# eazuooz/RayTracinginOneWeekendinCUDA

Measured on AMD Instinct MI355X. Metric: Msamples/s (pixels x spp / s), whole job, higher is better.
Workload: dtype f64; 1 GPU; C2 Book-1 final random-spheres, HittableList world (no BVH), 1200x800x500spp x50 bounces; frames_in_flight=1, width=1200, height=800, spp=500, max_depth=50, seed=1984, variant=strict, rng=XORWOW (cuRAND device-API semantics), one sequence per pixel

## Files before the change

### include/rtow.h

```cpp
#ifndef RTOW_H
#define RTOW_H

#include <stddef.h>
#include <stdint.h>

#ifdef __cplusplus
extern "C" {
#endif

#define RTOW_API __attribute__((visibility("default")))

typedef uint32_t rt_handle;
typedef struct rt_scene rt_scene;
typedef struct rt_rng rt_rng;
typedef struct rt_film rt_film;

enum rt_status {
    RT_OK = 0,
    RT_ERR_INVALID = 1,
    RT_ERR_UNSUPPORTED = 2,
    RT_ERR_HIP = 3,
    RT_ERR_NO_DEVICE = 4,
    RT_ERR_STATE = 5
};
// ... 73 lines not shown
    uint32_t n_nodes;
    uint32_t n_spheres, n_moving_spheres, n_quads;
    uint32_t n_objects;
    uint32_t n_xforms, n_media, n_materials, n_textures, n_perlin, n_images;
    uint32_t table_bytes;
    uint32_t image_bytes;
    uint32_t reserved[3];
} rt_scene_info;
RTOW_API int rt_scene_get_info(rt_scene *s, rt_scene_info *out);

RTOW_API int rt_scene_dump_leaves(rt_scene *s, int max_leaves, int *kind_out, double *box_out);
RTOW_API int rt_scene_dump_nodes(rt_scene *s, int max_nodes, double *box_out, uint32_t *abe_out);
RTOW_API int rt_scene_dump_fast_nodes(rt_scene *s, int max_nodes, double *box_out, uint32_t *ab_out, uint16_t *link_out);
RTOW_API int rt_scene_dump_camera(rt_scene *s, double out27[27]);
RTOW_API int rt_scene_dump_scan_segments(rt_scene *s, int max_segments, uint32_t *rows_axis_out, float *shared_out);

typedef struct rt_render_params {
    int32_t width, height;
    int32_t samples_per_pixel;
    int32_t max_depth;
    uint64_t seed;
    int32_t stripe_rows;
    int32_t rank, world_size;
    int32_t variant;
    int32_t device;
    int32_t flags;
    void *stream;
    int32_t coop_threshold;
    int32_t overdue_rays_per_sample;
    int32_t shade_batch;
    int32_t max_blocks_per_cu;
    int32_t pixels_per_wave;
    int32_t reserved0;
} rt_render_params;

#define RT_FLAG_KEEP_RNG_STATE 1u
#define RT_FLAG_OVERDUE_PRIORITY 4u
#define RT_FLAG_ACCUMULATE 8u
#define RT_FLAG_FORCE_GENERAL 2u
#define RT_FLAG_ALWAYS_WALK 32u
#define RT_FLAG_NO_PIXEL_CLASSES 64u
#define RT_FLAG_REFERENCE_TREE 128u
#define RT_FLAG_EXACT_SCAN 256u
#define RT_FLAG_FILTER_FP64 2048u
#define RT_FLAG_ACCELERATE_LISTS 512u
#define RT_FLAG_COOP_SINGLE 1024u
#define RT_FLAG_ROW_MAJOR_TILES 16u

typedef struct rt_render_stats {
    uint64_t samples;
    uint64_t rays;
    double seconds_seed;
    double seconds_render;
    uint32_t pixels;
    uint32_t rows;
    uint32_t kernel_vgprs;
    uint32_t lds_bytes;
    uint32_t kernel_kind;
    uint32_t pixels_per_wave;
// ... 158 lines not shown
```

### raytracinginoneweekendincuda_amd/__init__.py

```python
from .api import (
    RtowError,
    Rng,
    Scene,
    Film,
    RenderParams,
    RenderStats,
    LaunchPlan,
    builtin_scene,
    stripe_rows,
    deinterleave,
    write_ppm,
    write_ppm_binary,
    write_pfm,
    rtwimage_bytes,
    load_image,
    load_obj,
    jpeg_decode,
    library_path,
    lib,
    AdaptiveParams,
    adaptive_converged,
    adaptive_rule_on_device,
    FLAG_KEEP_RNG_STATE,
    FLAG_FORCE_GENERAL,
    FLAG_OVERDUE_PRIORITY,
    FLAG_ACCUMULATE,
    FLAG_ROW_MAJOR_TILES,
    FLAG_ALWAYS_WALK, FLAG_NO_PIXEL_CLASSES, FLAG_REFERENCE_TREE, FLAG_EXACT_SCAN, FLAG_ACCELERATE_LISTS, FLAG_COOP_SINGLE, FLAG_FILTER_FP64,
    SCENE_PLAIN_QUADS, SCENE_REFERENCE_TREE_ONLY,
)

__all__ = [
    "RtowError", "Rng", "Scene", "Film", "RenderParams", "RenderStats", "builtin_scene",
    "stripe_rows", "deinterleave", "write_ppm", "write_ppm_binary", "write_pfm", "rtwimage_bytes", "load_image", "load_obj", "library_path", "lib",
    "FLAG_KEEP_RNG_STATE", "FLAG_FORCE_GENERAL", "FLAG_OVERDUE_PRIORITY", "FLAG_ACCUMULATE", "FLAG_ROW_MAJOR_TILES", "FLAG_ALWAYS_WALK",
    "AdaptiveParams", "adaptive_converged", "adaptive_rule_on_device",
]
```

### raytracinginoneweekendincuda_amd/_lib.py

```python
import ctypes as C
import os

_HERE = os.path.dirname(os.path.abspath(__file__))
LIB_PATH = os.environ.get("RTOW_LIB_PATH") or os.path.join(_HERE, "librtow_hip.so")


class RenderParams(C.Structure):
    _fields_ = [
        ("width", C.c_int32), ("height", C.c_int32), ("samples_per_pixel", C.c_int32), ("max_depth", C.c_int32),
        ("seed", C.c_uint64), ("stripe_rows", C.c_int32), ("rank", C.c_int32), ("world_size", C.c_int32),
        ("variant", C.c_int32), ("device", C.c_int32), ("flags", C.c_int32), ("stream", C.c_void_p),
        ("coop_threshold", C.c_int32), ("overdue_rays_per_sample", C.c_int32),
        ("shade_batch", C.c_int32), ("max_blocks_per_cu", C.c_int32), ("pixels_per_wave", C.c_int32), ("reserved0", C.c_int32),
    ]


class RenderStats(C.Structure):
    _fields_ = [
        ("samples", C.c_uint64), ("rays", C.c_uint64), ("seconds_seed", C.c_double), ("seconds_render", C.c_double),
        ("pixels", C.c_uint32), ("rows", C.c_uint32), ("kernel_vgprs", C.c_uint32), ("lds_bytes", C.c_uint32),
        ("kernel_kind", C.c_uint32), ("pixels_per_wave", C.c_uint32),
    ]


# ... 126 lines not shown
    "rt_hittable_list": (H, [P, C.POINTER(H), I]),
    "rt_constant_medium": (H, [P, H, D, D, D, D]),
    "rt_constant_medium_tex": (H, [P, H, D, H]),
    "rt_bvh_node": (H, [P, C.POINTER(H), I]),
    "rt_hittable_bounding_box": (I, [P, H, D3]),
    "rt_scene_set_world": (I, [P, H]),
    "rt_scene_set_camera": (I, [P, D3, D3, D3, D, D, D, D, D, D, D3]),
    "rt_scene_build_builtin": (I, [P, I, I, I, I, C.c_uint64, P, I, I]),
    "rt_scene_commit": (I, [P]),
    "rt_scene_get_info": (I, [P, C.POINTER(SceneInfo)]),
    "rt_scene_dump_leaves": (I, [P, I, C.POINTER(C.c_int), D3]),
    "rt_scene_dump_nodes": (I, [P, I, D3, C.POINTER(C.c_uint32)]),
    "rt_scene_dump_fast_nodes": (I, [P, I, D3, C.POINTER(C.c_uint32), C.POINTER(C.c_uint16)]),
    "rt_scene_dump_camera": (I, [P, D3]),
    "rt_scene_dump_scan_segments": (I, [P, I, C.POINTER(C.c_uint32), C.POINTER(C.c_float)]),
    "rt_stripe_rows": (I, [I, I, I, I, C.POINTER(C.c_int), I]),
    "rt_film_create": (P, [I, I, I, I, I, I]),
    "rt_film_destroy": (None, [P]),
    "rt_film_device_pixels": (P, [P]),
    "rt_film_pixel_bytes": (C.c_size_t, [P]),
    "rt_film_bind_pixels": (I, [P, P]),
    "rt_plan_launch": (I, [P, C.POINTER(RenderParams), I, I, C.POINTER(LaunchPlan)]),
    "rt_film_download_probe_costs": (I, [P, C.POINTER(C.c_uint32), I, I]),
    "rt_scene_upload": (I, [P, I]),
    "rt_render_launch": (I, [P, P, C.POINTER(RenderParams)]),
    "rt_render_finish": (I, [P, P, C.POINTER(RenderStats)]),
    "rt_film_download": (I, [P, D3, I, I]),
    "rt_film_set_adaptive": (I, [P, C.POINTER(AdaptiveParams)]),
    "rt_film_download_sample_counts": (I, [P, C.POINTER(C.c_uint32), I, I]),
    "rt_adaptive_converged": (I, [C.POINTER(AdaptiveParams), C.c_uint32, D, D, D, D]),
# ... 44 lines not shown
```

### raytracinginoneweekendincuda_amd/api.py

```python
import ctypes as C
import numbers

import numpy as np

from . import _lib
from ._lib import (AdaptiveParams, DenoiseParams, FeatureParams, LaunchPlan, QueryHits, QueryParams, QueryRays, QueryStats,
                   RadianceOut, RadianceParams, RadianceRays, RadianceStats, RenderParams, RenderStats, SceneInfo)


class RtowError(RuntimeError):
    pass


FLAG_KEEP_RNG_STATE = 1
FLAG_FORCE_GENERAL = 2
FLAG_OVERDUE_PRIORITY = 4
FLAG_ACCUMULATE = 8
FLAG_ROW_MAJOR_TILES = 16
FLAG_ALWAYS_WALK = 32
FLAG_ACCELERATE_LISTS = 512
FLAG_EXACT_SCAN = 256
FLAG_REFERENCE_TREE = 128
FLAG_FILTER_FP64 = 2048
FLAG_COOP_SINGLE = 1024
FLAG_NO_PIXEL_CLASSES = 64


SCENE_PLAIN_QUADS = 1
SCENE_REFERENCE_TREE_ONLY = 2


DENOISE_DEFAULTS = {"iterations": 5, "sigma_color": 0.6, "sigma_albedo": 0.1, "sigma_normal": 0.3, "sigma_depth": 0.1}


def lib():
    return _lib.load()


def library_path():
# ... 199 lines not shown
        return boxes[:n], ab[:n], links[:n]

    def dump_camera(self):
        out = np.zeros(27, dtype=np.float64)
        _check(lib().rt_scene_dump_camera(self._p, out.ctypes.data_as(_lib.D3)))
        return out

    def scan_segments(self):
        n = lib().rt_scene_dump_scan_segments(self._p, 0, None, None)
        if n < 0:
            raise RtowError(_err())
        rows = np.zeros((max(n, 1), 3), dtype=np.uint32)
        shared = np.zeros(max(n, 1), dtype=np.float32)
        lib().rt_scene_dump_scan_segments(self._p, n, rows.ctypes.data_as(C.POINTER(C.c_uint32)), shared.ctypes.data_as(C.POINTER(C.c_float)))
        return [(int(r[0]), int(r[1]), None if r[2] == 3 else int(r[2]), shared[k]) for k, r in enumerate(rows[:n])]

    def plan_launch(self, params, num_cus=256, adaptive=False):
        out = LaunchPlan()
        _check(lib().rt_plan_launch(self._p, C.byref(params), num_cus, 1 if adaptive else 0, C.byref(out)))
        plan = {n: getattr(out, n) for n, _ in LaunchPlan._fields_ if not n.startswith("lds_table_")}
        plan["lds_tables"] = {name: (None if off == _lib.LDS_GLOBAL else off, size)
                              for name, off, size in zip(_lib.LDS_TABLES, out.lds_table_offset, out.lds_table_bytes)}
        return plan

    def upload(self, device=0):
        _check(lib().rt_scene_upload(self._p, device))

    def _ray_batch(self, kind, origins, directions, inputs, outputs, want, calls, structs, stats, device):
        on_gpu = type(origins).__module__.split(".")[0] == "torch"
        if on_gpu:
# ... 322 lines not shown
```

### raytracinginoneweekendincuda_amd/csrc/device_scene.cpp

```cpp
#include <hip/hip_runtime.h>

#include <cstdio>
#include <cmath>
#include <cstring>
#include <initializer_list>
#include <map>
#include <mutex>
#include <string>
#include <vector>

#include "../../include/rtow.h"
#include "device_arena.h"
#include "film_rows.h"
#include "launch_plan.h"
#include "render_iface.h"
#include "scene_host.h"

namespace rtow {

static int hip_fail(hipError_t e, const char *what)
{
    return fail(RT_ERR_HIP, std::string("HIP error = ") + std::to_string((unsigned)e) + " (" + hipGetErrorString(e) +
                                ") at '" + what + "'");
}
#define HIP_TRY(expr)                                     \
    do {                                                  \
        hipError_t e_ = (expr);                           \
        if (e_ != hipSuccess) return hip_fail(e_, #expr); \
    } while (0)
// ... 44 lines not shown
    DeviceArena planes;
    size_t plane_pixels() const { return geometry.n_pixels ? geometry.n_pixels : 1; }
    double *pixels = nullptr;
    double *own_pixels = nullptr;
    double *accum = nullptr;
    int accum_spp = 0;
    double *carry = nullptr;
    uint32_t *state = nullptr;
    unsigned long long *ray_counter = nullptr;
    int num_cus = 256;
    hipStream_t own_stream = nullptr;
    hipStream_t last_stream = nullptr;
    uint32_t *tile_cost = nullptr, *tile_order = nullptr;
    uint32_t *pix_cost = nullptr, *heavy_list = nullptr, *heavy_count = nullptr, *super_list = nullptr;
    uint8_t *pix_class = nullptr;
    unsigned long long *host_counters = nullptr;
    hipEvent_t ev[4] = {nullptr, nullptr, nullptr, nullptr};
    bool seeded = false;
    bool in_flight = false;
    SceneImpl *scene_in_flight = nullptr;
    uint64_t last_samples = 0;
    int last_variant = 0;
    rt_launch_plan last_plan{};
    KernelInfo last_kernel{};
    bool adaptive = false, frame_adaptive = false, last_adaptive = false;
    AdaptiveRule rule{}, frame_rule{};
    uint32_t *ad_n = nullptr;
    double *ad_q = nullptr;
    uint8_t *ad_mark = nullptr;
    bool rendered = false;
// ... 273 lines not shown
    f->geometry = film_geometry(width, height, stripe_rows, rank, world_size);
    const size_t np = f->plane_pixels();
    hipError_t e = f->planes.alloc(np * 3, f->own_pixels);
    if (e == hipSuccess) e = hipMemset(f->own_pixels, 0, np * 3 * sizeof(double));
    f->pixels = f->own_pixels;
    if (e == hipSuccess) e = f->planes.alloc(np * 6, f->state);
    if (e == hipSuccess) e = f->planes.alloc(kCounterWords, f->ray_counter);
    if (e == hipSuccess) {
        hipDeviceProp_t prop;
        e = hipGetDeviceProperties(&prop, device);
        if (e == hipSuccess) f->num_cus = prop.multiProcessorCount;
    }
    if (e == hipSuccess) e = hipStreamCreateWithFlags(&f->own_stream, hipStreamNonBlocking);
    if (e == hipSuccess) e = f->planes.alloc(f->geometry.n_tiles, f->tile_cost);
    if (e == hipSuccess) e = f->planes.alloc(f->geometry.n_tiles, f->tile_order);
    if (e == hipSuccess) e = hipHostMalloc((void **)&f->host_counters, kCounterWords * sizeof(unsigned long long), hipHostMallocDefault);
    for (int k = 0; k < 4 && e == hipSuccess; k++) e = hipEventCreate(&f->ev[k]);
    if (e != hipSuccess) {
        hip_fail(e, "rt_film_create allocation");
        rt_film_destroy(reinterpret_cast<rt_film *>(f));
        return nullptr;
    }
    return reinterpret_cast<rt_film *>(f);
}

void rt_film_destroy(rt_film *film)
{
    if (!film) return;
    FilmImpl *f = F(film);
    hipSetDevice(f->device);
// ... 219 lines not shown
    HIP_TRY(hipEventRecord(f.ev[0], stream));
    if (!keep)
        if (int rc = seed_film(f, p, stream)) return rc;
    HIP_TRY(hipEventRecord(f.ev[1], stream));
    RenderArgs ra{};
    if (int rc = book_frame(f, p, keep, continues, ra, stream)) return rc;
    const rt_launch_plan plan = plan_launch(ds, f.geometry, f.num_cus, *p, f.adaptive, hits_stay_in_boxes(s.flat, s.camera, p->variant));
    fill_render_args(f, p, plan, ra);
    KernelInfo info{};
    HIP_TRY(build.info(plan.kernel, ds, ra, &info));
    if (info.kind != plan.kernel_kind || info.lds_bytes != plan.lds_bytes)
        return fail(RT_ERR_STATE, "rt_render_launch: the kernel is not the one the launch plan describes");
    f.last_plan = plan;
    f.last_kernel = info;
    if (int rc = allocate_class_planes(f, plan)) return rc;
    if (plan.probe_spp > 0)
        if (int rc = enqueue_rehearsal(f, ds, plan, build, ra, stream)) return rc;
    HIP_TRY(build.render(plan.kernel, ds, ra, stream));
    HIP_TRY(hipEventRecord(f.ev[2], stream));
    HIP_TRY(hipMemcpyAsync(f.host_counters, f.ray_counter, kCounterWords * sizeof(unsigned long long), hipMemcpyDeviceToHost, stream));
    HIP_TRY(hipEventRecord(f.ev[3], stream));
    return RT_OK;
}

int rt_render_launch(rt_scene *scene, rt_film *film, const rt_render_params *p)
{
    if (!scene || !film || !p) return fail(RT_ERR_INVALID, "rt_render_launch: null argument");
    SceneImpl &s = *S(scene);
    FilmImpl &f = *F(film);
    if (p->width != f.geometry.width || p->height != f.geometry.height || p->stripe_rows != f.stripe_rows || p->rank != f.rank ||
// ... 38 lines not shown
                            "box pass", "medium pass / between walks", "object pass", "primitive pass", "  hit record", "  scatter",
                            "  next camera ray", "  pixel done"};
    if (is_sphere_list_kernel(f.last_kernel.kind)) {
        name[0] = "scan, pixel-parallel";
        name[1] = "scan, cooperative";
        name[12] = name[13] = "";
        const double passes = (double)c[96 + 0], groups = (double)c[96 + 12], taken = (double)c[64 + 12];
        if (groups > 0) {
            std::fprintf(stderr, "survivors: %.0f passes, %.2f groups of 4 per pass, groups taken f = %.4f\n", passes, groups / passes, taken / groups);
            std::fprintf(stderr, "survivors: spheres with a passing lane per taken group %.3f, lane appends per pass %.1f, lanes behind per pass %.2f\n",
                         (double)c[32 + 12] / taken, (double)c[96 + 13] / passes, (double)c[64 + 13] / passes);
            std::fprintf(stderr, "survivors: drains per pass %.2f, drain iterations (wave max of count) per pass %.2f, drain cycles %.1f %% of the "
                         "pixel-parallel scan's (%.0f of %.0f per pass)\n", (double)c[96 + 15] / passes, (double)c[64 + 15] / passes,
                         100.0 * c[32 + 13] / c[32 + 0], (double)c[32 + 13] / passes, (double)c[32 + 0] / passes);
        }
        name[16] = name[17] = name[18] = "";
        const double gp = (double)c[96 + 16];
        if (gp > 0) {
            std::fprintf(stderr, "grouped: %.0f passes through the filter, %.2f rays per pass, exact-test blocks executed per pass %.2f\n", gp,
                         (double)c[64 + 16] / gp, (double)c[32 + 16] / gp);
            std::fprintf(stderr, "grouped: survivors (lanes tested) per pass %.2f, largest per-lane count per pass %.2f, drains per pass %.2f\n",
                         (double)c[32 + 17] / gp, (double)c[64 + 17] / gp, (double)c[96 + 17] / gp);
            std::fprintf(stderr, "grouped: cycles per pass: filter %.0f, exact tests %.0f (%.1f %% and %.1f %% of the cooperative scans' %.0f)\n",
                         (double)c[64 + 18] / gp, (double)c[32 + 18] / gp, 100.0 * c[64 + 18] / c[32 + 1], 100.0 * c[32 + 18] / c[32 + 1],
                         (double)c[32 + 1] / (double)c[96 + 1]);
        }
    }
    const double total = (double)c[7];
    for (int k = 0; k < 24; k++)
        if (name[k][0] && c[96 + k])
// ... 448 lines not shown
```

### raytracinginoneweekendincuda_amd/csrc/render.hip

```cpp
#include <hip/hip_runtime.h>

#include <cfloat>
#include <cstddef>
#include <cstdint>
#include <type_traits>

#include "flat_scene.h"
#include "launch_plan.h"
#include "render_iface.h"
#include "rng.h"

#ifndef RT_STRICT
#define RT_STRICT 1
#endif
#ifndef RT_GROUP
#define RT_GROUP 0
#endif
#ifndef RT_ADAPT
#define RT_ADAPT 0
#endif
#ifndef RT_FEATURES
#define RT_FEATURES 0
#endif
#ifndef RT_QUERY
// ... 1431 lines not shown
    const double bu = f.od - s;
    return bu > f.root_m && __builtin_fma(bu, bu, k - q) > 0.0;
}

DEV SphereScanRow load_scan_row(const SphereScanRow *table, uint32_t k)
{
    const RT_CONST double *p = const_doubles(table + k);
    return SphereScanRow{p[0], p[1], p[2], p[3]};
}
DEV void scan_rows_arrived(const SphereScanRow &g0, const SphereScanRow &g1, const SphereScanRow &g2, const SphereScanRow &g3)
{
    asm volatile("" ::"s"(g0.cx), "s"(g0.cy), "s"(g0.cz), "s"(g0.k), "s"(g1.cx), "s"(g1.cy), "s"(g1.cz), "s"(g1.k));
    asm volatile("" ::"s"(g2.cx), "s"(g2.cy), "s"(g2.cz), "s"(g2.k), "s"(g3.cx), "s"(g3.cy), "s"(g3.cz), "s"(g3.k));
}

constexpr int kFilterTrip = 8;
static_assert(kFilterTrip < kQueueCap, "a trip of appends must fit between the drain threshold and the end of the queue");
DEV void append_survivor(uint16_t *queue, uint32_t lane, uint32_t &count, uint32_t k, bool keep)
{
    queue[count * 64u + lane] = (uint16_t)k;
    count += keep ? 1u : 0u;
}

DEV void filter_four(const SphereScanRow &g0, const SphereScanRow &g1, const SphereScanRow &g2, const SphereScanRow &g3, uint32_t k0,
                     const ScanRay &f, uint16_t *queue, uint32_t lane, uint32_t &count)
{
    const SphereScanRow *g[4] = {&g0, &g1, &g2, &g3};
    double s[4], q[4];
#pragma unroll
    for (int u = 0; u < 4; u++) {
// ... 1357 lines not shown
    int i = 0, j = 0;
    size_t local = 0;
    Xorwow rng{0, 0, 0, 0, 0, 0};
    Vec col = mk(0.0, 0.0, 0.0);
    Vec throughput = mk(1.0, 1.0, 1.0), accumulated = mk(0.0, 0.0, 0.0);
    Ray ray{};
    int sample = 0, depth = 0;
    uint32_t wave_rays = 0;
    [[maybe_unused]] uint32_t ad_before = 0;
    [[maybe_unused]] double ad_q = 0.0;
    [[maybe_unused]] unsigned long long wave_samples = 0;

    uint32_t pix_rays = 0;
    uint32_t my_tile = 0;
    int boost_left = 0;
    Walk walk{};
    walk.state = kNone;
    HitInfo walk_best;
    walk_best.t = 0.0;
    walk_best.ref = kNone;
    walk_best.obj = kNone;
    [[maybe_unused]] SegState seg{0u, kSegEnd, 0u};

    const uint32_t probe_cap = (!T::ADAPTIVE && a.probe && a.probe_ray_cap > 0) ? (uint32_t)a.probe_ray_cap : 0xFFFFFFFFu;
    auto book_cost = [&](uint32_t rays) {
        if constexpr (T::PARK) {
            local = (size_t)park_get_int<T::BLOCK>(sc.lds_park, 2);
            const uint32_t row = (uint32_t)local / (uint32_t)a.width, column = (uint32_t)local % (uint32_t)a.width;
            my_tile = (row >> 3) * tiles_x + (column >> 3);
        }
// ... 4 lines not shown
#if RT_PHASES
    PhaseSums ph{};
    const unsigned long long ph_start = __builtin_readcyclecounter();
    bool ph_serving = heavy_mode;
#endif
    for (;;) {
        unsigned long long overdue = 0;
        bool boost = false;
        if constexpr (T::WORLD == 2) {
            overdue = __ballot(active && pix_rays >= a.ray_budget);
            if (a.overdue_priority) {
                if (overdue) __builtin_amdgcn_s_setprio(3);
                else __builtin_amdgcn_s_setprio(0);
                overdue = 0;
            }
            boost = overdue != 0 && boost_left > 0;
            if (boost) boost_left--;
            else boost_left = a.boost_rounds;
        }

        const bool from_list = heavy_mode && !heavy_dry;
        if (solo_hold && !__any(active)) solo_hold = false;
        if (!exhausted && !boost && (!heavy_mode || from_list) && !solo_hold) {
            unsigned long long need = __ballot(!active);
            const bool from_super = from_list && solo_phase;
            const int ppw = from_super ? super_ppw : (from_list ? heavy_ppw : a.pixels_per_wave);
            if (ppw < 64) need &= (1ull << ppw) - 1ull;
            if (need) {
                PH_BEGIN();
                [[maybe_unused]] const bool ph_was_idle = !active;
                const uint32_t cnt = (uint32_t)__popcll(need);
                const uint32_t queue_len = from_super ? super_total : (from_list ? heavy_total : total_slots);
                uint32_t base = 0;
// ... 90 lines not shown
#endif
                continue;
            }
            if (exhausted) break;
            continue;
        }

        unsigned long long todo = live;
        HitInfo h;
        h.t = 0.0;
        h.ref = kNone;
        h.obj = kNone;
        bool hit = false;
        if constexpr (T::WORLD == 2) {
            if (boost) todo = overdue;
            if (!boost && a.pixels_per_wave >= 64 && __popcll(live) >= a.coop_threshold) {
                PH_BEGIN();
#if RT_PHASES
                ScanSums ss{};
#endif
                if (active) hit = a.exact_scan    ? scan_uniform(sc, queue, lane, ray, 0.001, DBL_MAX, h)
                                 : a.filter_fp64 ? (sv.in_lds ? scan_filtered<true>(sc, sv.planes_off, sv.n_padded, queue, lane, ray, 0.001, DBL_MAX, h SS_PASS)
                                                              : scan_filtered<false>(sc, 0u, 0u, queue, lane, ray, 0.001, DBL_MAX, h SS_PASS))
                                 : sv.in_lds     ? scan_filtered32<true>(sc, sv.planes_off, sv.n_padded, queue, lane, ray, 0.001, DBL_MAX, h SS_PASS)
                                                 : scan_filtered32<false>(sc, 0u, 0u, queue, lane, ray, 0.001, DBL_MAX, h SS_PASS);
                PH_END(0, active);
#if RT_PHASES
                {
                    const int src = __ffsll((long long)__ballot(active)) - 1;
                    if (src >= 0) {
                    const auto rl = [src](uint32_t v) { return (unsigned long long)(uint32_t)__builtin_amdgcn_readlane((int)v, src); };
                    ph.n[12] += rl(ss.groups);  ph.l[12] += rl(ss.taken);        ph.t[12] += rl(ss.spheres);
                    ph.n[13] += rl(ss.appends); ph.l[13] += rl(ss.behind);       ph.t[13] += rl(ss.drain_cycles);
                    ph.n[15] += rl(ss.drains);  ph.l[15] += rl(ss.drain_iters);
                    }
                }
#endif
            } else {
                PH_BEGIN();
#if RT_PHASES
                GroupedSums gs{};
#endif
// ... 386 lines not shown
    klass[k] = heavy ? 1 : 0;
    if (longest) super_list[atomicAdd(count + 1, 1u)] = k;
    else if (heavy) list[atomicAdd(count, 1u)] = k;
}

hipError_t launch_classify_pixels(const uint32_t *pix_cost, uint32_t n_pixels, uint32_t threshold, uint8_t *pix_class, uint32_t *list,
                                  uint32_t *count, hipStream_t stream, uint32_t *super_list, uint32_t super_threshold, uint32_t width,
                                  uint32_t near_percent, uint32_t near_neighbours)
{
    if (n_pixels == 0) return hipSuccess;
    hipLaunchKernelGGL(classify_pixels_kernel, dim3((n_pixels + 255u) / 256u), dim3(256), 0, stream, pix_cost, n_pixels, threshold,
                       pix_class, list, count, super_list, super_threshold, width, near_percent, near_neighbours);
    return hipGetLastError();
}

hipError_t launch_tile_order(const uint32_t *tile_cost, uint32_t *tile_order, uint32_t n_tiles, uint32_t flat_x8, hipStream_t stream)
{
    if (n_tiles == 0) return hipSuccess;
    hipLaunchKernelGGL(tile_order_kernel, dim3(1), dim3(1024), 0, stream, tile_cost, tile_order, n_tiles, flat_x8);
    return hipGetLastError();
}
#endif

#if RT_STRICT
#define RT_SUFFIX strict
#else
#define RT_SUFFIX fast
#endif
#define RT_CAT2(a, b) a##b
#define RT_CAT(a, b) RT_CAT2(a, b)
// ... 581 lines not shown
```

### raytracinginoneweekendincuda_amd/csrc/render_iface.h

```cpp
#pragma once
#include <hip/hip_runtime.h>

#include <cstdint>

#include "adaptive_rule.h"
#include "flat_scene.h"
#include "rng.h"

namespace rtow {

struct SeedArgs {
    uint32_t *state;
    const uint32_t *jump_table;
    Xorwow base;
    uint32_t *tile_cost;
    const uint32_t *tile_order;
    int32_t probe;
    uint32_t n_pixels;
    int32_t width, stripe_rows, rank, world_size;
};

struct RenderArgs {
    double *pixels;
    double *accum;
// ... 32 lines not shown
    int32_t exact_scan;
    int32_t filter_fp64;
    int32_t reference_tree;
    int32_t always_walk;
    int32_t force_general;
    int32_t coop_threshold;
    int32_t coop_single;
    int32_t num_cus;
    int32_t lds_spheres;
    int32_t overdue_priority;
    int32_t boost_rounds;
    int32_t max_blocks_per_cu;
    int32_t pixels_per_wave;
    int32_t shade_batch;
    uint32_t ray_budget;
    int32_t adaptive;
    AdaptiveRule rule;
    uint32_t *ad_n;
    double *ad_q;
    uint8_t *ad_mark;
};

struct KernelInfo {
    int vgprs, lds_bytes, kind;
};

hipError_t launch_seed_strict(const SeedArgs &a, hipStream_t stream);
hipError_t launch_seed_fast(const SeedArgs &a, hipStream_t stream);
hipError_t launch_render_strict(int kernel, const DeviceScene &sc, const RenderArgs &a, hipStream_t stream);
hipError_t launch_render_fast(int kernel, const DeviceScene &sc, const RenderArgs &a, hipStream_t stream);
// ... 59 lines not shown

struct AtrousArgs {
    const double *in;
    double *out;
    const double *albedo, *normal;
    const double *depth;
    int32_t width, height, step;
    double inv_color, inv_albedo, inv_normal, inv_depth;
};
hipError_t launch_atrous(const AtrousArgs &a, hipStream_t stream);

hipError_t launch_classify_pixels(const uint32_t *pix_cost, uint32_t n_pixels, uint32_t threshold, uint8_t *pix_class, uint32_t *list,
                                  uint32_t *count, hipStream_t stream, uint32_t *super_list = nullptr, uint32_t super_threshold = 0,
                                  uint32_t width = 0, uint32_t near_percent = 0, uint32_t near_neighbours = 0);

hipError_t launch_tile_order(const uint32_t *tile_cost, uint32_t *tile_order, uint32_t n_tiles, uint32_t flat_x8, hipStream_t stream);

}
```

### raytracinginoneweekendincuda_amd/csrc/scene_builder.cpp

```cpp
#include <algorithm>
#include <cfloat>
#include <charconv>
#include <cmath>
#include <limits>
#include <cstdio>
#include <cstdlib>
#include <cstring>
#include <mutex>
#include <unordered_map>

#include "../../include/rtow.h"
#include "scene_host.h"

namespace rtow {

static thread_local std::string g_error;
void set_error(const std::string &msg) { g_error = msg; }
int fail(int status, const std::string &msg)
{
    g_error = msg;
    return status;
}

static inline D3 mk(double x, double y, double z) { return D3{x, y, z}; }
static inline D3 add(D3 a, D3 b) { return mk(a.x + b.x, a.y + b.y, a.z + b.z); }
static inline D3 sub(D3 a, D3 b) { return mk(a.x - b.x, a.y - b.y, a.z - b.z); }
// ... 2044 lines not shown
    if (!s || !S(s)->committed) return -fail(RT_ERR_STATE, "rt_scene_dump_scan_segments: scene not committed");
    const FlatScene &f = S(s)->flat;
    const int n = (int)f.scan_segments.size();
    for (int k = 0; k < n && k < max_segments; k++) {
        const ScanSegment &sg = f.scan_segments[k];
        if (rows_axis_out) {
            rows_axis_out[3 * k] = sg.first_trip * 2u * kScanTripPairs;
            rows_axis_out[3 * k + 1] = sg.n_trips * 2u * kScanTripPairs;
            rows_axis_out[3 * k + 2] = sg.axis;
        }
        if (shared_out) shared_out[k] = sg.c;
    }
    return n;
}

int rt_stripe_rows(int height, int stripe_rows, int rank, int world_size, int *rows_out, int max_rows)
{
    if (height < 0 || stripe_rows <= 0 || world_size <= 0 || rank < 0 || rank >= world_size) return -1;
    int n = 0;
    for (int j = 0; j < height; j++)
        if ((j / stripe_rows) % world_size == rank) {
            if (rows_out && n < max_rows) rows_out[n] = j;
            n++;
        }
    return n;
}

int rt_deinterleave(const double *gathered, int width, int height, int stripe_rows, int world_size,
                    size_t rank_stride_doubles, double *frame_full)
{
// ... 75 lines not shown
```

Measured before the change: 3064 Msamples/s.

## Cull camera rays against per-tile sphere lists built from conservative view cones

Adds a pre-pass kernel that builds, for each 8x8 tile, a conservative cone covering all camera rays (including lens defocus), and lists up to 14 spheres that can intersect it. In the sphere-list render kernel, depth-0 rays for fresh lanes test only their tile's list instead of the full sphere scan, skipping most of the 485-sphere intersection work for primary rays. Tiles whose cone intersects too many spheres fall back to the full scan, and the path is gated by a break-even estimate and a disable flag. It adds an extra kernel launch, more branching and register pressure in the main kernel, and depends on the culling bounds being conservative for bit-exact results.

Result: faster. 3351 Msamples/s, median of 6 (+9.4%).

```diff
diff --git a/include/rtow.h b/include/rtow.h
--- a/include/rtow.h
+++ b/include/rtow.h
@@ -111,6 +111,8 @@
 RTOW_API int rt_scene_dump_fast_nodes(rt_scene *s, int max_nodes, double *box_out, uint32_t *ab_out, uint16_t *link_out);
 RTOW_API int rt_scene_dump_camera(rt_scene *s, double out27[27]);
 RTOW_API int rt_scene_dump_scan_segments(rt_scene *s, int max_segments, uint32_t *rows_axis_out, float *shared_out);
+RTOW_API int rt_scene_dump_primary_lists(rt_scene *s, int width, int height, int stripe_rows, int rank, int world_size, int max_tiles,
+                                         uint16_t *lists_out);
 
 typedef struct rt_render_params {
     int32_t width, height;
@@ -140,6 +142,7 @@
 #define RT_FLAG_REFERENCE_TREE 128u
 #define RT_FLAG_EXACT_SCAN 256u
 #define RT_FLAG_FILTER_FP64 2048u
+#define RT_FLAG_NO_PRIMARY_LISTS 4096u
 #define RT_FLAG_ACCELERATE_LISTS 512u
 #define RT_FLAG_COOP_SINGLE 1024u
 #define RT_FLAG_ROW_MAJOR_TILES 16u
diff --git a/profiles/primary_lists_measure.py b/profiles/primary_lists_measure.py
--- /dev/null
+++ b/profiles/primary_lists_measure.py
@@ -0,0 +1,66 @@
+import argparse
+import os
+import sys
+
+import numpy as np
+
+sys.path.insert(0, os.path.join(os.path.dirname(os.path.abspath(__file__)), ".."))
+import raytracinginoneweekendincuda_amd as rt
+
+
+def random_y_list():
+    src = rt.builtin_scene(11, 1, 600, 400)
+    _, boxes = src.dump_leaves()
+    centres, radii = 0.5 * (boxes[:, 0::2] + boxes[:, 1::2]), 0.5 * (boxes[:, 1] - boxes[:, 0])
+    rnd = np.random.default_rng(13)
+    s = rt.Scene()
+    items = []
+    for k, (c, r) in enumerate(zip(centres, radii)):
+        y = float(c[1]) if r > 10 else float(rnd.uniform(0.2, 3.0))
+        mat = s.Dielectric(1.5) if k % 9 == 0 else (s.Metal((0.7, 0.6, 0.5), 0.1) if k % 4 == 0 else s.Lambertian((0.2 + 0.05 * (k % 12), 0.4, 0.6)))
+        items.append(s.Sphere((float(c[0]), y, float(c[2])), float(r), mat))
+    s.SetWorld(s.HittableList(items))
+    s.Camera((13.0, 2.0, 3.0), (0.0, 0.0, 0.0), (0, 1, 0), 20.0, 600 / 400, 0.1, 10.0)
+    s.Commit()
+    return s
+
+
+def measure(name, scene, w, h, spp, frames):
+    times = {0: [], rt.FLAG_NO_PRIMARY_LISTS: []}
+    out = {}
+    kind = None
+    for k in range(frames + 1):
+        for flags in (rt.FLAG_NO_PRIMARY_LISTS, 0):
+            film = rt.Film(w, h)
+            st = film.render(scene, spp, flags=flags)
+            kind = st.kernel_kind
+            if k:
+                times[flags].append(st.seconds_render * 1e3)
+            out[flags] = film.download().copy()
+    on, off = np.array(times[0]), np.array(times[rt.FLAG_NO_PRIMARY_LISTS])
+    lists = scene.primary_lists(w, h)
+    lens = [len(l) for l in lists if l is not None]
+    print("%-28s kind %3d  off %8.3f ms (%.3f-%.3f)  on %8.3f ms (%.3f-%.3f)  %+6.1f %%  frames equal: %s  lists: %d of %d tiles, mean %.2f" % (
+        name, kind, np.median(off), off.min(), off.max(), np.median(on), on.min(), on.max(), 100.0 * (np.median(on) / np.median(off) - 1.0),
+        np.array_equal(out[0].view(np.uint64), out[rt.FLAG_NO_PRIMARY_LISTS].view(np.uint64)), len(lens), len(lists), float(np.mean(lens)) if lens else 0.0), flush=True)
+
+
+def main():
+    ap = argparse.ArgumentParser()
+    ap.add_argument("--frames", type=int, default=5)
+    args = ap.parse_args()
+    w, h = 600, 400
+    for scene_id in range(12):
+        try:
+            s = rt.builtin_scene(scene_id, 1, w, h)
+        except rt.RtowError:
+            continue
+        plan = s.plan_launch(rt.RenderParams(w, h, 50, 50, 1984, 8, 0, 1, 0, 0, 0, None, 0, 0, 0, 0, 0, 0))
+        if plan["kernel_kind"] != 16:
+            continue
+        measure("scene %d, 50 spp" % scene_id, s, w, h, 50, args.frames)
+    measure("485 spheres, random y, 200 spp", random_y_list(), w, h, 200, args.frames)
+
+
+if __name__ == "__main__":
+    main()
diff --git a/raytracinginoneweekendincuda_amd/__init__.py b/raytracinginoneweekendincuda_amd/__init__.py
--- a/raytracinginoneweekendincuda_amd/__init__.py
+++ b/raytracinginoneweekendincuda_amd/__init__.py
@@ -27,6 +27,7 @@
     FLAG_ACCUMULATE,
     FLAG_ROW_MAJOR_TILES,
     FLAG_ALWAYS_WALK, FLAG_NO_PIXEL_CLASSES, FLAG_REFERENCE_TREE, FLAG_EXACT_SCAN, FLAG_ACCELERATE_LISTS, FLAG_COOP_SINGLE, FLAG_FILTER_FP64,
+    FLAG_NO_PRIMARY_LISTS,
     SCENE_PLAIN_QUADS, SCENE_REFERENCE_TREE_ONLY,
 )
 
diff --git a/raytracinginoneweekendincuda_amd/_lib.py b/raytracinginoneweekendincuda_amd/_lib.py
--- a/raytracinginoneweekendincuda_amd/_lib.py
+++ b/raytracinginoneweekendincuda_amd/_lib.py
@@ -164,6 +164,7 @@
     "rt_scene_dump_fast_nodes": (I, [P, I, D3, C.POINTER(C.c_uint32), C.POINTER(C.c_uint16)]),
     "rt_scene_dump_camera": (I, [P, D3]),
     "rt_scene_dump_scan_segments": (I, [P, I, C.POINTER(C.c_uint32), C.POINTER(C.c_float)]),
+    "rt_scene_dump_primary_lists": (I, [P, I, I, I, I, I, I, C.POINTER(C.c_uint16)]),
     "rt_stripe_rows": (I, [I, I, I, I, C.POINTER(C.c_int), I]),
     "rt_film_create": (P, [I, I, I, I, I, I]),
     "rt_film_destroy": (None, [P]),
diff --git a/raytracinginoneweekendincuda_amd/api.py b/raytracinginoneweekendincuda_amd/api.py
--- a/raytracinginoneweekendincuda_amd/api.py
+++ b/raytracinginoneweekendincuda_amd/api.py
@@ -23,6 +23,7 @@
 FLAG_REFERENCE_TREE = 128
 FLAG_FILTER_FP64 = 2048
 FLAG_COOP_SINGLE = 1024
+FLAG_NO_PRIMARY_LISTS = 4096
 FLAG_NO_PIXEL_CLASSES = 64
 
 
@@ -252,6 +253,14 @@
         shared = np.zeros(max(n, 1), dtype=np.float32)
         lib().rt_scene_dump_scan_segments(self._p, n, rows.ctypes.data_as(C.POINTER(C.c_uint32)), shared.ctypes.data_as(C.POINTER(C.c_float)))
         return [(int(r[0]), int(r[1]), None if r[2] == 3 else int(r[2]), shared[k]) for k, r in enumerate(rows[:n])]
+
+    def primary_lists(self, width, height, stripe_rows=8, rank=0, world_size=1):
+        n = lib().rt_scene_dump_primary_lists(self._p, width, height, stripe_rows, rank, world_size, 0, None)
+        if n < 0:
+            raise RtowError(_err())
+        words = np.zeros((max(n, 1), 16), dtype=np.uint16)
+        lib().rt_scene_dump_primary_lists(self._p, width, height, stripe_rows, rank, world_size, n, words.ctypes.data_as(C.POINTER(C.c_uint16)))
+        return [None if w[0] == 15 else [int(k) for k in w[1:1 + int(w[0])]] for w in words[:n]]
 
     def plan_launch(self, params, num_cus=256, adaptive=False):
         out = LaunchPlan()
diff --git a/raytracinginoneweekendincuda_amd/csrc/device_scene.cpp b/raytracinginoneweekendincuda_amd/csrc/device_scene.cpp
--- a/raytracinginoneweekendincuda_amd/csrc/device_scene.cpp
+++ b/raytracinginoneweekendincuda_amd/csrc/device_scene.cpp
@@ -13,6 +13,7 @@
 #include "device_arena.h"
 #include "film_rows.h"
 #include "launch_plan.h"
+#include "primary_cull_rule.h"
 #include "render_iface.h"
 #include "scene_host.h"
 
@@ -87,6 +88,7 @@
     uint32_t *tile_cost = nullptr, *tile_order = nullptr;
     uint32_t *pix_cost = nullptr, *heavy_list = nullptr, *heavy_count = nullptr, *super_list = nullptr;
     uint8_t *pix_class = nullptr;
+    uint16_t *primary_lists = nullptr;
     unsigned long long *host_counters = nullptr;
     hipEvent_t ev[4] = {nullptr, nullptr, nullptr, nullptr};
     bool seeded = false;
@@ -390,6 +392,7 @@
     if (e == hipSuccess) e = hipStreamCreateWithFlags(&f->own_stream, hipStreamNonBlocking);
     if (e == hipSuccess) e = f->planes.alloc(f->geometry.n_tiles, f->tile_cost);
     if (e == hipSuccess) e = f->planes.alloc(f->geometry.n_tiles, f->tile_order);
+    if (e == hipSuccess) e = f->planes.alloc((size_t)f->geometry.n_tiles * kPrimaryListWords, f->primary_lists);
     if (e == hipSuccess) e = hipHostMalloc((void **)&f->host_counters, kCounterWords * sizeof(unsigned long long), hipHostMallocDefault);
     for (int k = 0; k < 4 && e == hipSuccess; k++) e = hipEventCreate(&f->ev[k]);
     if (e != hipSuccess) {
@@ -639,6 +642,12 @@
     f.last_plan = plan;
     f.last_kernel = info;
     if (int rc = allocate_class_planes(f, plan)) return rc;
+    if (is_sphere_list_kernel(plan.kernel_kind) && p->max_depth > 0 && !(p->flags & (RT_FLAG_EXACT_SCAN | RT_FLAG_NO_PRIMARY_LISTS)) &&
+        plan.pixels_per_wave >= 64 && plan.coop_threshold <= 64 && ds.n_spheres <= 0xFFFFu && f.geometry.n_tiles > 0) {
+        HIP_TRY(launch_primary_lists(ds, f.primary_lists, f.geometry.n_tiles, f.geometry.width, f.geometry.height, f.geometry.rows_owned,
+                                     f.stripe_rows, f.rank, f.world_size, stream));
+        ra.primary_lists = f.primary_lists;
+    }
     if (plan.probe_spp > 0)
         if (int rc = enqueue_rehearsal(f, ds, plan, build, ra, stream)) return rc;
     HIP_TRY(build.render(plan.kernel, ds, ra, stream));
@@ -707,6 +716,15 @@
                          "pixel-parallel scan's (%.0f of %.0f per pass)\n", (double)c[96 + 15] / passes, (double)c[64 + 15] / passes,
                          100.0 * c[32 + 13] / c[32 + 0], (double)c[32 + 13] / passes, (double)c[32 + 0] / passes);
         }
+        name[19] = "";
+        if (c[96 + 19])
+            std::fprintf(stderr, "camera rays: %llu pixel-parallel passes, %.2f live lanes per pass, %.2f of them with a camera ray (depth 0): share %.4f\n",
+                         c[96 + 19], (double)c[64 + 19] / c[96 + 19], (double)c[32 + 19] / c[96 + 19], (double)c[32 + 19] / (double)c[64 + 19]);
+        name[23] = "";
+        if (c[96 + 23])
+            std::fprintf(stderr, "primary: %llu rounds, %.2f fresh lanes per round, %.2f list entries tested per round (%.2f per lane), %.0f cycles per round "
+                         "(%.1f %% of wave time)\n", c[96 + 23], (double)c[64 + 23] / c[96 + 23], (double)c[32 + 15] / c[96 + 23],
+                         (double)c[32 + 15] / (double)c[64 + 23], (double)c[32 + 23] / c[96 + 23], 100.0 * c[32 + 23] / (double)c[7]);
         name[16] = name[17] = name[18] = "";
         const double gp = (double)c[96 + 16];
         if (gp > 0) {
diff --git a/raytracinginoneweekendincuda_amd/csrc/primary_cull_rule.h b/raytracinginoneweekendincuda_amd/csrc/primary_cull_rule.h
--- /dev/null
+++ b/raytracinginoneweekendincuda_amd/csrc/primary_cull_rule.h
@@ -0,0 +1,118 @@
+#pragma once
+#include <cstdint>
+
+#include "flat_scene.h"
+
+#if defined(__HIPCC__) || defined(__HIP__)
+#define RT_CULL_FN __host__ __device__ inline
+#else
+#define RT_CULL_FN inline
+#endif
+
+namespace rtow {
+
+constexpr uint32_t kPrimaryListWords = 16;
+constexpr uint32_t kPrimaryListMax = 14;
+constexpr uint32_t kPrimaryNoList = 15;
+
+struct TilePixels {
+    int32_t i0, i1, j0, j1;
+};
+
+RT_CULL_FN TilePixels primary_tile_pixels(uint32_t tile, int32_t width, int32_t rows_owned, int32_t stripe_rows, int32_t rank, int32_t world_size)
+{
+    const uint32_t tiles_x = ((uint32_t)width + 7u) >> 3;
+    const int32_t tx = (int32_t)(tile % tiles_x), ty = (int32_t)(tile / tiles_x);
+    TilePixels t;
+    t.i0 = tx * 8;
+    t.i1 = tx * 8 + 7 < width ? tx * 8 + 7 : width - 1;
+    const int32_t lr0 = ty * 8, lr1 = ty * 8 + 7 < rows_owned ? ty * 8 + 7 : rows_owned - 1;
+    t.j0 = 0x7fffffff;
+    t.j1 = -1;
+    for (int32_t lr = lr0; lr <= lr1; lr++) {
+        const int32_t j = ((lr / stripe_rows) * world_size + rank) * stripe_rows + (lr % stripe_rows);
+        t.j0 = j < t.j0 ? j : t.j0;
+        t.j1 = j > t.j1 ? j : t.j1;
+    }
+    return t;
+}
+
+struct TileCone {
+    double ax, ay, az;
+    double mx, my, mz;
+    double rho_a, k;
+    double mm, kk;
+    double a_norm;
+    bool open;
+};
+
+RT_CULL_FN double cull_norm3(double x, double y, double z) { return __builtin_sqrt(x * x + y * y + z * z); }
+
+RT_CULL_FN TileCone primary_tile_cone(const CameraRec &c, int32_t width, int32_t height, const TilePixels &t)
+{
+#if defined(__clang__)
+#pragma clang fp contract(off)
+#endif
+    const double s0 = (double)(t.i0 - 1) / (double)width, s1 = (double)(t.i1 + 2) / (double)width;
+    const double t0 = (double)(t.j0 - 1) / (double)height, t1 = (double)(t.j1 + 2) / (double)height;
+    const double sc = 0.5 * (s0 + s1), tc = 0.5 * (t0 + t1), hs = 0.5 * (s1 - s0), ht = 0.5 * (t1 - t0);
+    TileCone k;
+    k.ax = c.origin[0]; k.ay = c.origin[1]; k.az = c.origin[2];
+    k.mx = c.llc[0] + sc * c.horizontal[0] + tc * c.vertical[0] - k.ax;
+    k.my = c.llc[1] + sc * c.horizontal[1] + tc * c.vertical[1] - k.ay;
+    k.mz = c.llc[2] + sc * c.horizontal[2] + tc * c.vertical[2] - k.az;
+    const double uu = c.u[0] * c.u[0] + c.u[1] * c.u[1] + c.u[2] * c.u[2], vv = c.v[0] * c.v[0] + c.v[1] * c.v[1] + c.v[2] * c.v[2];
+    const double uv = c.u[0] * c.v[0] + c.u[1] * c.v[1] + c.u[2] * c.v[2];
+    const double smax = __builtin_sqrt(0.5 * ((uu + vv) + __builtin_sqrt((uu - vv) * (uu - vv) + 4.0 * (uv * uv))));
+    const double lens = c.lens_radius < 0.0 ? -c.lens_radius : c.lens_radius;
+    k.a_norm = cull_norm3(k.ax, k.ay, k.az);
+    const double scale = k.a_norm + cull_norm3(c.llc[0], c.llc[1], c.llc[2]) + cull_norm3(c.horizontal[0], c.horizontal[1], c.horizontal[2]) +
+                         cull_norm3(c.vertical[0], c.vertical[1], c.vertical[2]) + lens * (__builtin_sqrt(uu) + __builtin_sqrt(vv));
+    const double slack = 0x1p-40 * scale;
+    const double plus = cull_norm3(hs * c.horizontal[0] + ht * c.vertical[0], hs * c.horizontal[1] + ht * c.vertical[1], hs * c.horizontal[2] + ht * c.vertical[2]);
+    const double minus = cull_norm3(hs * c.horizontal[0] - ht * c.vertical[0], hs * c.horizontal[1] - ht * c.vertical[1], hs * c.horizontal[2] - ht * c.vertical[2]);
+    k.rho_a = (lens * smax) * (1.0 + 0x1p-40) + slack;
+    const double rho_b = (plus > minus ? plus : minus) * (1.0 + 0x1p-40) + slack;
+    k.k = k.rho_a + rho_b;
+    k.mm = k.mx * k.mx + k.my * k.my + k.mz * k.mz;
+    k.kk = k.k * k.k;
+    k.open = k.mm - k.kk > 0x1p-40 * (k.mm + k.kk);
+    return k;
+}
+
+RT_CULL_FN bool primary_may_hit(const TileCone &k, double cx, double cy, double cz, double r2)
+{
+#if defined(__clang__)
+#pragma clang fp contract(off)
+#endif
+    if (!k.open) return true;
+    const double c_norm = cull_norm3(cx, cy, cz);
+    const double reach = k.a_norm + k.rho_a + c_norm + __builtin_sqrt(r2);
+    const double q = __builtin_sqrt(r2 + 0x1p-40 * (reach * reach)) + k.rho_a;
+    const double wx = k.ax - cx, wy = k.ay - cy, wz = k.az - cz;
+    const double wc = k.a_norm + c_norm;
+    const double n0 = wc * wc + q * q, n2 = k.mm + k.kk;
+    const double c0 = (wx * wx + wy * wy + wz * wz) - q * q;
+    const double b1 = (wx * k.mx + wy * k.my + wz * k.mz) - q * k.k;
+    const double a2 = k.mm - k.kk;
+    const bool clear = c0 > 0x1p-40 * n0 && (b1 >= 0.0 || c0 * a2 - b1 * b1 > 0x1p-40 * (n0 * n2));
+    return !clear;
+}
+
+inline void primary_list_for_tile(const TileCone &k, const SphereGeom *spheres, uint32_t n_spheres, uint16_t out[kPrimaryListWords])
+{
+    for (uint32_t w = 0; w < kPrimaryListWords; w++) out[w] = 0;
+    uint32_t count = 0;
+    for (uint32_t s = 0; s < n_spheres && count <= kPrimaryListMax; s++) {
+        if (!primary_may_hit(k, spheres[s].cx, spheres[s].cy, spheres[s].cz, spheres[s].r2)) continue;
+        if (count < kPrimaryListMax) out[1 + count] = (uint16_t)s;
+        count++;
+    }
+    if (count > kPrimaryListMax) {
+        for (uint32_t w = 0; w < kPrimaryListWords; w++) out[w] = 0;
+        count = kPrimaryNoList;
+    }
+    out[0] = (uint16_t)count;
+}
+
+}
diff --git a/raytracinginoneweekendincuda_amd/csrc/render.hip b/raytracinginoneweekendincuda_amd/csrc/render.hip
--- a/raytracinginoneweekendincuda_amd/csrc/render.hip
+++ b/raytracinginoneweekendincuda_amd/csrc/render.hip
@@ -7,6 +7,7 @@
 
 #include "flat_scene.h"
 #include "launch_plan.h"
+#include "primary_cull_rule.h"
 #include "render_iface.h"
 #include "rng.h"
 
@@ -1469,6 +1470,8 @@
     asm volatile("" ::"s"(g2.cx), "s"(g2.cy), "s"(g2.cz), "s"(g2.k), "s"(g3.cx), "s"(g3.cy), "s"(g3.cz), "s"(g3.k));
 }
 
+constexpr uint32_t kPrimaryRoundCost = 735, kPrimaryPassFixed = 1200, kPrimaryPassPerSphere100 = 354;
+constexpr uint32_t kPrimaryLongChain = 6;
 constexpr int kFilterTrip = 8;
 static_assert(kFilterTrip < kQueueCap, "a trip of appends must fit between the drain threshold and the end of the queue");
 DEV void append_survivor(uint16_t *queue, uint32_t lane, uint32_t &count, uint32_t k, bool keep)
@@ -2856,6 +2859,9 @@
     uint32_t pix_rays = 0;
     uint32_t my_tile = 0;
     int boost_left = 0;
+    [[maybe_unused]] bool primary_since_scan = false;
+    [[maybe_unused]] const int primary_break_even = (int)((64u * kPrimaryRoundCost) / (kPrimaryPassFixed + (sc.n_spheres * kPrimaryPassPerSphere100) / 100u));
+    [[maybe_unused]] bool primary_last = false;
     Walk walk{};
     walk.state = kNone;
     HitInfo walk_best;
@@ -2890,9 +2896,14 @@
                 else __builtin_amdgcn_s_setprio(0);
                 overdue = 0;
             }
-            boost = overdue != 0 && boost_left > 0;
-            if (boost) boost_left--;
-            else boost_left = a.boost_rounds;
+            if (primary_last) {
+                overdue = 0;
+            } else {
+                boost = overdue != 0 && boost_left > 0;
+                if (boost) boost_left--;
+                else boost_left = a.boost_rounds;
+            }
+            primary_last = false;
         }
 
         const bool from_list = heavy_mode && !heavy_dry;
@@ -3013,7 +3024,78 @@
         bool hit = false;
         if constexpr (T::WORLD == 2) {
             if (boost) todo = overdue;
-            if (!boost && a.pixels_per_wave >= 64 && __popcll(live) >= a.coop_threshold) {
+            const bool scan_wave = !boost && a.pixels_per_wave >= 64 && __popcll(live) >= a.coop_threshold;
+            if (scan_wave && a.primary_lists != nullptr && a.max_depth > 0) {
+                const bool camera = active && depth == 0;
+                const unsigned long long cameras = __ballot(camera);
+                const bool may_round = !primary_since_scan && __popcll(cameras) >= primary_break_even &&
+                                       !__any(active && pix_rays > kPrimaryLongChain * (uint32_t)(sample + 16));
+                if (cameras == live || may_round) {
+                    PH_BEGIN();
+                    uint4 wa = uint4{kPrimaryNoList, 0u, 0u, 0u};
+                    const uint4 *row = reinterpret_cast<const uint4 *>(a.primary_lists + (size_t)my_tile * kPrimaryListWords);
+                    if (camera) wa = row[0];
+                    uint32_t n_listed = wa.x & 0xFFFFu;
+                    const bool fresh = camera && n_listed != kPrimaryNoList;
+                    const unsigned long long freshes = __ballot(fresh);
+                    primary_last = freshes != 0 && (freshes == live || (may_round && __popcll(freshes) >= primary_break_even));
+                    if (primary_last) primary_since_scan = true;
+                    if (primary_last) {
+                        todo = freshes;
+                        if (!fresh) n_listed = 0u;
+                        n_listed = n_listed < kPrimaryListMax ? n_listed : kPrimaryListMax;
+                        const double ra = dot(ray.d, ray.d);
+                        double closest = DBL_MAX;
+                        uint32_t best_k = kNone;
+#if RT_PHASES
+                        ph.n[23] += 1ull;
+                        ph.l[23] += (unsigned long long)__popcll(freshes);
+                        for (uint32_t e = n_listed, off = 32; off > 0; off >>= 1) {
+                            e += (uint32_t)__shfl_xor((int)e, (int)off, 64);
+                            if (off == 1) ph.t[15] += e;
+                        }
+#endif
+                        for (uint32_t s = 0; __any(s < n_listed); s++) {
+                            if (s == 7u) {
+                                if (s < n_listed) wa = row[1];
+                            } else {
+                                wa.x = __builtin_amdgcn_alignbit(wa.y, wa.x, 16); wa.y = __builtin_amdgcn_alignbit(wa.z, wa.y, 16);
+                                wa.z = __builtin_amdgcn_alignbit(wa.w, wa.z, 16); wa.w >>= 16;
+                            }
+                            if (s < n_listed) {
+                                const uint32_t k = wa.x & 0xFFFFu;
+                                SphereGeom g;
+                                if (sv.in_lds) {
+                                    const RT_LDS double *pl = (const RT_LDS double *)(lds_raw + sv.planes_off);
+                                    g = SphereGeom{pl[k], pl[sv.n_padded + k], pl[2u * sv.n_padded + k], pl[3u * sv.n_padded + k]};
+                                } else {
+                                    g = sc.spheres[k];
+                                }
+                                double t;
+                                if (sphere_test(ray.o - mk(g.cx, g.cy, g.cz), ray.d, ra, g.r2, 0.001, closest, t)) {
+                                    closest = t;
+                                    best_k = k;
+                                }
+                            }
+                        }
+                        hit = best_k != kNone;
+                        if (hit) {
+                            h.t = closest;
+                            h.ref = make_ref(REF_SPHERE, best_k);
+                            h.obj = kNone;
+                        }
+                    }
+#if RT_PHASES
+                    if (primary_last) {
+                        asm volatile("" ::"v"(h.t), "v"(h.ref));
+                        ph.t[23] += __builtin_readcyclecounter() - ph_t0;
+                    }
+#endif
+                }
+            }
+            if (primary_last) {
+            } else if (scan_wave) {
+                primary_since_scan = false;
                 PH_BEGIN();
 #if RT_PHASES
                 ScanSums ss{};
@@ -3025,6 +3107,9 @@
                                                  : scan_filtered32<false>(sc, 0u, 0u, queue, lane, ray, 0.001, DBL_MAX, h SS_PASS);
                 PH_END(0, active);
 #if RT_PHASES
+                ph.n[19] += 1ull;
+                ph.l[19] += (unsigned long long)__popcll(live);
+                ph.t[19] += (unsigned long long)__popcll(__ballot(active && depth == 0));
                 {
                     const int src = __ffsll((long long)__ballot(active)) - 1;
                     if (src >= 0) {
@@ -3441,6 +3526,48 @@
     return hipGetLastError();
 }
 
+__global__ __launch_bounds__(256) void primary_lists_kernel(DeviceScene sc, uint16_t *lists, uint32_t n_tiles, int32_t width, int32_t height,
+                                                             int32_t rows_owned, int32_t stripe_rows, int32_t rank, int32_t world_size)
+{
+    const uint32_t tile = blockIdx.x * blockDim.x + threadIdx.x;
+    if (tile >= n_tiles) return;
+    const CameraRec cam = *sc.camera;
+    const TileCone cone = primary_tile_cone(cam, width, height, primary_tile_pixels(tile, width, rows_owned, stripe_rows, rank, world_size));
+    uint32_t w[kPrimaryListWords / 2] = {0u, 0u, 0u, 0u, 0u, 0u, 0u, 0u};
+    uint32_t count = 0;
+    const uint32_t n = sc.n_spheres;
+    for (uint32_t s = 0; s < n; s++) {
+        const SphereGeom g = load_sphere_row(sc.spheres, s);
+        if (!primary_may_hit(cone, g.cx, g.cy, g.cz, g.r2)) continue;
+        if (count < kPrimaryListMax) {
+            const uint32_t slot = count + 1u;
+#pragma unroll
+            for (uint32_t q = 0; q < kPrimaryListWords / 2; q++)
+                if (q == slot / 2u) w[q] |= s << ((slot & 1u) * 16u);
+        }
+        count++;
+    }
+    if (count > kPrimaryListMax) {
+#pragma unroll
+        for (uint32_t q = 0; q < kPrimaryListWords / 2; q++) w[q] = 0u;
+        count = kPrimaryNoList;
+    }
+    w[0] |= count;
+    uint4 *out = reinterpret_cast<uint4 *>(lists + (size_t)tile * kPrimaryListWords);
+    out[0] = uint4{w[0], w[1], w[2], w[3]};
+    out[1] = uint4{w[4], w[5], w[6], w[7]};
+}
+
+hipError_t launch_primary_lists(const DeviceScene &sc, uint16_t *lists, uint32_t n_tiles, int32_t width, int32_t height, int32_t rows_owned,
+                                int32_t stripe_rows, int32_t rank, int32_t world_size, hipStream_t stream)
+{
+    if (n_tiles == 0) return hipSuccess;
+    if (sc.n_spheres > 0xFFFFu) return hipErrorInvalidValue;
+    hipLaunchKernelGGL(primary_lists_kernel, dim3((n_tiles + 255u) / 256u), dim3(256), 0, stream, sc, lists, n_tiles, width, height, rows_owned,
+                       stripe_rows, rank, world_size);
+    return hipGetLastError();
+}
+
 hipError_t launch_tile_order(const uint32_t *tile_cost, uint32_t *tile_order, uint32_t n_tiles, uint32_t flat_x8, hipStream_t stream)
 {
     if (n_tiles == 0) return hipSuccess;
diff --git a/raytracinginoneweekendincuda_amd/csrc/render_iface.h b/raytracinginoneweekendincuda_amd/csrc/render_iface.h
--- a/raytracinginoneweekendincuda_amd/csrc/render_iface.h
+++ b/raytracinginoneweekendincuda_amd/csrc/render_iface.h
@@ -70,6 +70,7 @@
     int32_t pixels_per_wave;
     int32_t shade_batch;
     uint32_t ray_budget;
+    const uint16_t *primary_lists;
     int32_t adaptive;
     AdaptiveRule rule;
     uint32_t *ad_n;
@@ -159,6 +160,9 @@
                                   uint32_t *count, hipStream_t stream, uint32_t *super_list = nullptr, uint32_t super_threshold = 0,
                                   uint32_t width = 0, uint32_t near_percent = 0, uint32_t near_neighbours = 0);
 
+hipError_t launch_primary_lists(const DeviceScene &sc, uint16_t *lists, uint32_t n_tiles, int32_t width, int32_t height, int32_t rows_owned,
+                                int32_t stripe_rows, int32_t rank, int32_t world_size, hipStream_t stream);
+
 hipError_t launch_tile_order(const uint32_t *tile_cost, uint32_t *tile_order, uint32_t n_tiles, uint32_t flat_x8, hipStream_t stream);
 
 }
diff --git a/raytracinginoneweekendincuda_amd/csrc/scene_builder.cpp b/raytracinginoneweekendincuda_amd/csrc/scene_builder.cpp
--- a/raytracinginoneweekendincuda_amd/csrc/scene_builder.cpp
+++ b/raytracinginoneweekendincuda_amd/csrc/scene_builder.cpp
@@ -10,6 +10,8 @@
 #include <unordered_map>
 
 #include "../../include/rtow.h"
+#include "launch_plan.h"
+#include "primary_cull_rule.h"
 #include "scene_host.h"
 
 namespace rtow {
@@ -2084,6 +2086,22 @@
     return n;
 }
 
+int rt_scene_dump_primary_lists(rt_scene *s, int width, int height, int stripe_rows, int rank, int world_size, int max_tiles, uint16_t *lists_out)
+{
+    if (!s || !S(s)->committed || !S(s)->has_camera) return -fail(RT_ERR_STATE, "rt_scene_dump_primary_lists: scene not committed, or no camera");
+    if (width <= 0 || height <= 0 || stripe_rows <= 0 || world_size <= 0 || rank < 0 || rank >= world_size)
+        return -fail(RT_ERR_INVALID, "rt_scene_dump_primary_lists: bad geometry");
+    const FlatScene &f = S(s)->flat;
+    if (f.spheres.size() > 0xFFFFu) return -fail(RT_ERR_INVALID, "rt_scene_dump_primary_lists: more spheres than a list entry can name");
+    const FilmGeometry g = film_geometry(width, height, stripe_rows, rank, world_size);
+    for (uint32_t tile = 0; tile < g.n_tiles && (int)tile < max_tiles; tile++) {
+        if (!lists_out) break;
+        const TileCone cone = primary_tile_cone(S(s)->camera, width, height, primary_tile_pixels(tile, width, g.rows_owned, stripe_rows, rank, world_size));
+        primary_list_for_tile(cone, f.spheres.data(), (uint32_t)f.spheres.size(), lists_out + (size_t)tile * kPrimaryListWords);
+    }
+    return (int)g.n_tiles;
+}
+
 int rt_stripe_rows(int height, int stripe_rows, int rank, int world_size, int *rows_out, int max_rows)
 {
     if (height < 0 || stripe_rows <= 0 || world_size <= 0 || rank < 0 || rank >= world_size) return -1;
```
